# MathThyMod/GP_emu_UQSA

Measured on AMD Instinct MI355X. Metric: log-marginal-likelihood evals/sec at n=16384 d=10 fp64; 1/2/4/8 GPU, higher is better.
Workload: dtype f64

## Files before the change

gp_emu_uqsa_amd/csrc/gpemu.hip:

```cpp
#include <hip/hip_runtime.h>

#include <algorithm>
#include <array>
#include <atomic>
#include <map>
#include <cmath>
#include <cstdio>
#include <cstdlib>
#include <cstring>
#include <limits>
#include <string>
#include <vector>

#include "../../include/gpemu.h"
#include "gpemu_kernels.hpp"
#include "gpemu_gemm_sched.hpp"
#include "gpemu_small.hpp"
#include "gpemu_tiny.hpp"
#include "gpemu_snb.hpp"
#include "gpemu_ozaki.hpp"
#include "gpemu_pivchol.hpp"
#include "gpemu_postgrad.hpp"
#include "gpemu_postmean.hpp"
#include "gpemu_postgroup.hpp"
// ... 11 lines not shown

enum AdhocSlot {
  ADHOC_POST_V = ADHOC_DESC_BASE + 0,
  ADHOC_COV = ADHOC_DESC_BASE + 1,
  ADHOC_NOISE = ADHOC_DESC_BASE + 3,
  ADHOC_PIVCHOL = ADHOC_DESC_BASE + 4,
  ADHOC_POST_U = ADHOC_DESC_BASE + 5,
  ADHOC_TEST = ADHOC_DESC_BASE + 8,
  ADHOC_BENCH = ADHOC_DESC_BASE + 16,
};

struct Plan {
  long long n_pad = 0;
  const double* a_ptr = nullptr;
  const double* b_ptr = nullptr;
  std::vector<int> fused, fused_aug;
  std::vector<int> trtri;
  std::vector<std::vector<std::array<int, 3>>> tri_pairs;
  int lauum = -1;
  bool aug = false;
  std::vector<int> grp, grp_aug;
  int split_h = 0, aug_mid = -1;
  std::vector<int> sfused, sfused_aug, sgrp, sgrp_aug;
  std::vector<GemmLaunch> launches;
  std::vector<GemmProb> probs;
  std::vector<unsigned> tiles;
};

constexpr int FACT_FLAG_INTS = 6;

constexpr int OZ_CHOL_MIN = 8192;


struct Fact {
  long long n_pad = 0;
  int NB = 0;
  double* A = nullptr;
  double* B = nullptr;
  size_t cap = 0;
  double* logdet = nullptr;
  int* flags = nullptr;
  int* tflags = nullptr;
  bool aug = false;
  double* Faug = nullptr;
  double* part = nullptr;
  int* tcnt = nullptr;
  bool xdone = false;
  int desc_base = 0;
  Plan plan;
};

}

struct gpe_ctx {
  int device = 0;
  hipStream_t stream = nullptr;
  std::string err;

  long long n = 0, n_pad = 0;
  int d = 0, q = 0, NB = 0;
  bool has_r = false;

  double* dX = nullptr;
  double* dXw = nullptr;
  double* dF = nullptr;
  double* dr = nullptr;
  Fact tr;
  Fact aux;

  int* dinfo = nullptr;
// ... 26 lines not shown
  double* dtiny = nullptr;
  int tiny_ek = 0, tiny_eg = 0;
  bool tiny_dirty = true;
  double* dsnb = nullptr;
  long long snb_np = 0;
  int snb_hc = 0, snb_mf = 0;
  bool snb_dirty = true;
  double onel_tag = 0.0;
  int oz_on = 1, oz_nmod = OZ_MAXMOD;
  int oz_min_np = 6144;
  int oz_np2 = 0, oz_list_len = 0;
  long long oz_npad = 0;
  OzConst oz_c{};
  int8_t* dozp = nullptr;
  int8_t* dozr = nullptr;
  int* dozx = nullptr;
  unsigned* dozl = nullptr;
  double* dozt = nullptr;
  hipEvent_t ev_oz = nullptr;
  std::vector<OzTriPair> oz_tri;
  int oz_tri_min = 8192;
  double oz_lauum_ops = 0.0;
  int oz_chol = 1, oz_chol_min = OZ_CHOL_MIN;
  OzTriPair oz_chol_q{};
  long long oz_chol_loff = 0;
  int oz_chol_llen = 0;
  double oz_chol_ops = 0.0;
  bool oz_chol_ready = false;
  bool oz_l21_valid = false;
  std::vector<hipEvent_t> oev;
  size_t oev_used = 0;
  double oz_ms = 0.0, oz_launches = 0.0, oz_ops = 0.0, oz_flops64 = 0.0;
  int dbg_skip_wait = -1;
  size_t small_cap = 0;

  double* hpin = nullptr;
  size_t hpin_cap = 0;

  float* dX32 = nullptr;
  size_t x32_cap = 0;
  bool x32_valid = false;
  float* dK32 = nullptr;
  size_t k32_cap = 0;
  hipEvent_t ev_pipe[2] = {nullptr, nullptr};
  int8_t* dpxp = nullptr;
  int* dpxe = nullptr;
// ... 620 lines not shown
        }
        if (i < base.size()) order.push_back(base[i]);
      }
      auto move_to = [&](unsigned code, size_t at) {
        const auto it = std::find(order.begin(), order.end(), code);
        order.erase(it);
        order.insert(order.begin() + std::min(at, order.size()), code);
      };
      if (!rest0.empty() && order.size() > 256 + head) {
        const auto it = std::find(order.begin(), order.end(), rest0.front());
        if ((size_t)(it - order.begin()) > 255 + head) move_to(rest0.front(), 255 + head);
      }
      if (!waits_point_back(fp.data(), order))
        return fail(c, GPE_ERR_HIP, "internal error: group schedule waits on a later tile");
      gidx[o + gb] = (int)pl.launches.size();
      add_launch(pl, GEMM_FUSED, fp, fl, &order);
      pl.launches.back().ticket = flags0 + 3 * NB + gb;
    }
  }
  }
  return GPE_OK;
  };
  CHK(sweep(0, NB, NB, {&pl.fused, &pl.fused_aug, &pl.grp, &pl.grp_aug}));
  for (int s = 2; s / 2 < NB; s *= 2) {
    std::vector<GemmProb> pa, pb;
    const std::vector<std::array<int, 3>> prs = trtri_level_pairs(NB, s);
    double fa = 0.0, fb = 0.0;
    for (const auto& pr : prs) {
      const int t0 = pr[0], h = pr[1], t1 = pr[2];
      const int a = h - t0, b = t1 - h;
      pa.push_back(mkprob(tile(B, t0, t0), ld, tile(A, h, t0), ld, tile(B, t0, h), ld, a, b,
                          a * TILE, G_KBEG_TI, 1.0, 0.0));
      fa += (double)a * T * a * T * b * T;
      pb.push_back(mkprob(tile(B, h, h), ld, tile(B, t0, h), ld, tile(B, h, t0), ld, b, a,
                          b * TILE, G_KEND_TI, -1.0, 0.0));
      fb += (double)b * T * b * T * a * T;
    }
    if (pa.empty()) continue;
    pl.tri_pairs.push_back(prs);
    split_k(pa, F.part, F.tcnt);
    split_k(pb, F.part, F.tcnt);
    pl.trtri.push_back((int)pl.launches.size());
    add_launch(pl, GEMM_AK, pa, fa);
    pl.trtri.push_back((int)pl.launches.size());
    add_launch(pl, GEMM_PLAIN, pb, fb);
  }
  pl.lauum = (int)pl.launches.size();
  {
    const double N = (double)F.n_pad;
    std::vector<GemmProb> lp = {mkprob(B, ld, B, ld, A, ld, NB, NB, (int)F.n_pad, G_CLOWER | G_KBEG_TI, 1.0, 0.0)};
    split_k(lp, F.part, F.tcnt);
    add_launch(pl, GEMM_AK_BK, lp, N * N * N / 3.0);
  }
  const int limit = (F.desc_base == 0) ? AUX_DESC_BASE : ADHOC_DESC_BASE - AUX_DESC_BASE;
  if (const int h = (&F == &c->tr) ? oz_chol_split(c, F) : 0) {
    const size_t nl = pl.launches.size(), np = pl.probs.size(), nt = pl.tiles.size();
    pl.sfused.assign(NB, -1);
    pl.sfused_aug.assign(NB, -1);
    if (c->potrf_group) {
      pl.sgrp.assign(NB, -1);
      if (pl.aug) pl.sgrp_aug.assign(NB, -1);
    }
    const std::array<std::vector<int>*, 4> ix = {&pl.sfused, &pl.sfused_aug, &pl.sgrp, &pl.sgrp_aug};
    CHK(sweep(0, h, NB, ix));
    CHK(sweep(h, NB - h, NB - h, ix));
    if (pl.aug) {
      pl.aug_mid = (int)pl.launches.size();
      add_launch(pl, GEMM_PLAIN, {mkprob(F.Faug, TILE, tile(A, h, 0), ld, F.Faug + (long long)h * TILE * TILE, TILE, 1, NB - h,
                                h * TILE, 0, -1.0, 1.0)}, 0.0);
    }
    pl.split_h = h;
    if ((int)pl.probs.size() > limit) {
      pl.launches.resize(nl);
      pl.probs.resize(np);
      pl.tiles.resize(nt);
      pl.split_h = 0;
      pl.aug_mid = -1;
    }
  }
  if ((int)pl.probs.size() > limit) return fail(c, GPE_ERR_UNSUPPORTED, "GEMM schedule too large");
  for (auto& L : pl.launches) L.first += F.desc_base;
  HIPCHK(c, hipMemcpy(c->dprobs + F.desc_base, pl.probs.data(), pl.probs.size() * sizeof(GemmProb),
                      hipMemcpyHostToDevice));
  const size_t half = pl.tiles.size() + 1;
  const size_t need = 2 * half;
  const bool regrow = need > c->tiles_cap;
  CHK(grow_buf(c, &c->dtiles, &c->tiles_cap, need));
  if (regrow) {
    Fact& other = (&F == &c->tr) ? c->aux : c->tr;
    other.plan = Plan();
  }
  const size_t base = (F.desc_base == 0) ? 0 : c->tiles_cap / 2;
  if (pl.tiles.size() > c->tiles_cap / 2) return fail(c, GPE_ERR_STATE, "tile list overflow");
  for (auto& L : pl.launches)
    if (L.list >= 0) L.list += (long long)base;
  if (!pl.tiles.empty())
    HIPCHK(c, hipMemcpy(c->dtiles + base, pl.tiles.data(), pl.tiles.size() * sizeof(unsigned),
                        hipMemcpyHostToDevice));
  return GPE_OK;
}
// ... 56 lines not shown
    *coff = 1.0;
    *cdiag = predict ? 1.0 + nu * nu : 1.0;
  } else {
    *coff = 1.0 - nu;
    *cdiag = predict ? 1.0 : 1.0 - nu;
  }
}

int kbuild(gpe_ctx* c, int kernel, double nu, double s2, double rscale) {
  PairArgs a;
  a.xr = c->dXw; a.xc = c->dXw; a.out = c->tr.A; a.ld = c->n_pad;
  a.d = c->d; a.nr_valid = (int)c->n; a.nc_valid = (int)c->n;
  a.mt = c->NB; a.nt = c->NB; a.mode = 1 | 2;
  double coff, cdiag;
  kernel_consts(kernel, nu, true, &coff, &cdiag);
  a.s2 = s2; a.coff = coff; a.cdiag = cdiag;
  a.rscale = rscale; a.r = (c->has_r && rscale != 0.0) ? c->dr : nullptr;
  a.fam = kernel_fam(kernel);
  return launch_pairs(c, a, c->NB * (c->NB + 1) / 2);
}

int oz_prepare(gpe_ctx* c, Fact& F);
int chol_schur(gpe_ctx* c, Fact& F, hipStream_t st, bool with_aug);

int potrf(gpe_ctx* c, Fact& F, bool with_aug = false, bool split = false) {
  CHK(build_plan(c, F));
  const int hs = split ? F.plan.split_h : 0;
  if (hs) CHK(oz_prepare(c, F));
  const Plan& pl = F.plan;
  if (hs != (split ? pl.split_h : 0)) return fail(c, GPE_ERR_STATE, "internal error: split plan changed");
  const int NB = F.NB;
  HIPCHK(c, hipMemsetAsync(F.flags, 0, FACT_FLAG_INTS * (size_t)NB * sizeof(int), c->stream));
  F.xdone = false;
  const bool wa = with_aug && pl.aug;
  const bool grp = c->potrf_group &&
                   (c->potrf_mode == 1 || (c->potrf_mode == 0 && g_inflight[c->device & 63].load() <= 1));
  const std::vector<int>& fidx = hs ? (grp ? (wa ? pl.sgrp_aug : pl.sgrp) : (wa ? pl.sfused_aug : pl.sfused))
                                    : (grp ? (wa ? pl.grp_aug : pl.grp) : (wa ? pl.fused_aug : pl.fused));
  if (c->chol_prio) {
    HIPCHK(c, hipEventRecord(c->ev_fork, c->stream));
    HIPCHK(c, hipStreamWaitEvent(c->stream2, c->ev_fork, 0));
    for (int t = 0; t < NB; ++t) {
      if (hs && t == hs) CHK(chol_schur(c, F, c->stream2, wa));
      if (fidx[t] >= 0) CHK(launch_gemm_range(c, pl.launches[fidx[t]], c->stream2));
    }
    HIPCHK(c, hipEventRecord(c->ev_join, c->stream2));
    HIPCHK(c, hipStreamWaitEvent(c->stream, c->ev_join, 0));
    return GPE_OK;
  }
#ifdef GEMM_TTRACE
  if (const char* es = std::getenv("GPEMU_DEBUG_STOP_STEP")) {
    const int stop = std::atoi(es);
    for (int t = 0; t <= stop && t < NB; ++t)
      if (fidx[t] >= 0) CHK(launch_gemm_range(c, pl.launches[fidx[t]]));
    HIPCHK(c, hipStreamSynchronize(c->stream));
    return fail(c, GPE_ERR_STATE, "debug stop after Cholesky launch " + std::to_string(stop));
  }
#endif
  for (int t = 0; t < NB; ++t) {
    if (hs && t == hs) CHK(chol_schur(c, F, c->stream, wa));
    if (fidx[t] >= 0) CHK(launch_gemm_range(c, pl.launches[fidx[t]]));
  }
  return GPE_OK;
}

void ev_rec(gpe_ctx* c, int i);

int lauum(gpe_ctx* c, Fact& F) {
  CHK(build_plan(c, F));
  return launch_gemm_range(c, F.plan.launches[F.plan.lauum]);
}

int ensure_xdiag(gpe_ctx* c, Fact& F) {
  if (F.xdone) return GPE_OK;
  hipLaunchKernelGGL(k_xasm, dim3(F.NB), dim3(256), DB_LDS_DOUBLES * sizeof(double), c->stream, F.A, F.B,
                     (long long)F.n_pad);
  HIPCHK(c, hipGetLastError());
  F.xdone = true;
  return GPE_OK;
}

int trtri_pair_ozaki(gpe_ctx* c, Fact& F, int t0, int h, int t1, int l21);
int oz_l21_ahead(gpe_ctx* c, Fact& F, int t0, int h, int t1);
bool oz_tri_level(const gpe_ctx* c, const std::vector<std::array<int, 3>>& prs);

int trtri(gpe_ctx* c, Fact& F, bool ozaki = false) {
  CHK(build_plan(c, F));
  CHK(ensure_xdiag(c, F));
  const Plan& pl = F.plan;
  int first = -1;
  for (size_t lv = 0; lv < pl.tri_pairs.size() && ozaki && first < 0; ++lv)
    if (oz_tri_level(c, pl.tri_pairs[lv])) first = (int)lv;
  bool have = false;
  if (first >= 0) {
    const auto& pr = pl.tri_pairs[first][0];
    have = c->oz_l21_valid && &F == &c->tr && pl.split_h > 0 && pr[0] == 0 && pr[1] == pl.split_h && pr[2] == F.NB;
    if (!have) CHK(oz_l21_ahead(c, F, pr[0], pr[1], pr[2]));
  }
  for (size_t lv = 0; lv < pl.tri_pairs.size(); ++lv) {
    if (ozaki && oz_tri_level(c, pl.tri_pairs[lv])) {
      for (size_t i = 0; i < pl.tri_pairs[lv].size(); ++i) {
        const auto& pr = pl.tri_pairs[lv][i];
        CHK(trtri_pair_ozaki(c, F, pr[0], pr[1], pr[2], ((int)lv == first && i == 0) ? (have ? 2 : 1) : 0));
      }
      continue;
    }
    CHK(launch_gemm_range(c, pl.launches[pl.trtri[2 * lv]]));
    CHK(launch_gemm_range(c, pl.launches[pl.trtri[2 * lv + 1]]));
  }
  return GPE_OK;
}

int skinny(gpe_ctx* c, bool transposed, const double* M, long long ldm, int ntr, int nit,
           bool lower, const double* R, long long ldr, int P, double* Y, long long ldy) {
  if (P > SK_PMAX) {
    for (int c0 = 0; c0 < P; c0 += SK_PMAX)
      CHK(skinny(c, transposed, M, ldm, ntr, nit, lower, R + (long long)c0 * ldr, ldr, std::min(SK_PMAX, P - c0),
                 Y + (long long)c0 * ldy, ldy));
    return GPE_OK;
  }
  const int kext = lower ? std::max(ntr, nit) : ntr;
  const int want = (256 + nit - 1) / nit;
  const int chk = std::max(1, std::min(SK_CH, (kext + want - 1) / want));
  const int nch = (kext + chk - 1) / chk;
  const long long rows = (long long)nit * TILE;
  CHK(grow_buf(c, &c->dskp, &c->skp_cap, (size_t)nch * rows * P));
  SkinnyArgs a;
  a.M = M; a.ldm = ldm; a.R = R; a.ldr = ldr; a.part = c->dskp; a.ldp = rows;
  a.pstride = rows * P; a.P = P; a.ntr = ntr; a.lower = lower ? 1 : 0; a.nit = nit;
  a.abort_flag = c->dinfo;
  a.chk = chk;
  dim3 grid(nit * nch);
// ... 122 lines not shown
int z_from_factor(gpe_ctx* c);
int trsv_lower(gpe_ctx* c, Fact& F, const double* R, long long ldr, int P, double* Y, long long ldy);

int factor_and_invert(gpe_ctx* c, int kernel, const double* delta, double nu, double s2,
                      double rscale, bool invert = true, bool objective = false) {
  c->linv_valid = false;
  c->oz_l21_valid = false;
  HIPCHK(c, hipStreamSynchronize(c->stream2));
  HIPCHK(c, hipMemsetAsync(c->dinfo, 0, sizeof(int), c->stream));
  CHK(build_plan(c, c->tr));
  ev_rec(c, 0);
  CHK(scale_training(c, delta));
  CHK(kbuild(c, kernel, nu, s2, rscale));
  const int P = c->q + 1;
  c->zaug_valid = !invert && c->tr.plan.aug && P <= TILE;
  if (c->zaug_valid) {
    const long long tot = c->n_pad * TILE;
    hipLaunchKernelGGL(k_aug_init, dim3((unsigned)((tot + 255) / 256)), dim3(256), 0, c->stream, c->dF,
                       c->n_pad, P, c->n_pad, c->tr.Faug);
    HIPCHK(c, hipGetLastError());
  }
  ev_rec(c, 1);
  CHK(build_plan(c, c->tr));
  CHK(potrf(c, c->tr, c->zaug_valid, objective && (invert || c->oz_chol >= 2)));
  if (kernel_fam(kernel) != FAM_GAUSS) {
    double coff, cdiag;
    kernel_consts(kernel, nu, true, &coff, &cdiag);
    const double floor_rel = 4.0 * (double)c->n_pad * std::numeric_limits<double>::epsilon();
    const double* r = (c->has_r && rscale != 0.0) ? c->dr : nullptr;
    hipLaunchKernelGGL(k_pivot_floor, dim3((unsigned)((c->n + 255) / 256)), dim3(256), 0, c->stream, c->tr.A,
                       c->n_pad, (int)c->n, floor_rel, s2 * cdiag, r, rscale, c->dinfo);
    HIPCHK(c, hipGetLastError());
  }
  ev_rec(c, 2);
  if (invert) {
    CHK(trtri(c, c->tr, true));
    c->linv_valid = true;
  }
  CHK(z_from_factor(c));
  ev_rec(c, 3);
  return GPE_OK;
}

int z_from_factor(gpe_ctx* c) {
  const int P = c->q + 1;
  const long long np = c->n_pad;
  if (c->zaug_valid) {
// ... 159 lines not shown
  return nullptr;
}

int oz_l21(gpe_ctx* c, Fact& F, const OzTriPair& q, hipStream_t st) {
  c->oz_l21_valid = false;
  oz_operand(st, c->oz_c, q.l21(F.A + (long long)q.h * TILE + (long long)q.t0 * TILE * F.n_pad, F.n_pad), q.Pb, q.Pa,
             c->dozx, c->dozp);
  HIPCHK(c, hipGetLastError());
  return GPE_OK;
}

int oz_l21_ahead(gpe_ctx* c, Fact& F, int t0, int h, int t1) {
  CHK(oz_prepare(c, F));
  const OzTriPair* q = oz_pair(c, t0, h, t1);
  if (!q) return fail(c, GPE_ERR_STATE, "internal error: TRTRI pair without an int8 plan");
  if (!c->ev_oz) HIPCHK(c, hipEventCreateWithFlags(&c->ev_oz, hipEventDisableTiming));
  HIPCHK(c, hipEventRecord(c->ev_fork, c->stream));
  HIPCHK(c, hipStreamWaitEvent(c->stream2, c->ev_fork, 0));
  CHK(oz_l21(c, F, *q, c->stream2));
  HIPCHK(c, hipEventRecord(c->ev_oz, c->stream2));
  return GPE_OK;
}

int trtri_pair_ozaki(gpe_ctx* c, Fact& F, int t0, int h, int t1, int l21) {
  CHK(oz_prepare(c, F));
  const OzTriPair* qp = oz_pair(c, t0, h, t1);
  if (!qp) return fail(c, GPE_ERR_STATE, "internal error: TRTRI pair without an int8 plan");
  const long long ld = F.n_pad;
  auto tile = [&](double* M, int i, int j) { return M + (long long)i * TILE + (long long)j * TILE * ld; };
  if (l21 == 1) HIPCHK(c, hipStreamWaitEvent(c->stream, c->ev_oz, 0));
  c->oz_l21_valid = false;
  int rc = GPE_OK;
  oz_tri_pair_launches(c->stream, c->oz_c, *qp, c->dozl, tile(F.A, h, t0), tile(F.B, t0, t0), tile(F.B, h, h),
                       tile(F.B, h, t0), ld, c->dozt, c->dozp, c->dozr, c->dozx, l21 != 0,
                       [&](const OzProduct& p, double ops, double fl) {
                         if (rc == GPE_OK) rc = oz_gemm_crt(c, c->oz_c, p, ops, fl);
                       });
  CHK(rc);
  HIPCHK(c, hipGetLastError());
  return GPE_OK;
}

}

bool create_priority_stream(hipStream_t* st) {
  int lo = 0, hi = 0;
  if (hipDeviceGetStreamPriorityRange(&lo, &hi) != hipSuccess) return false;
  return hipStreamCreateWithPriority(st, hipStreamNonBlocking, hi) == hipSuccess;
}

extern "C" {

#ifdef GEMM_TRACE
int gpe_debug_trace(uint64_t* out, int32_t n) {
  if (n > 8 * 4096) n = 8 * 4096;
  return hipMemcpyFromSymbol(out, HIP_SYMBOL(gemm_trace), (size_t)n * 8) == hipSuccess ? 0 : -2;
}
#endif

#ifdef GEMM_TTRACE
// ... 50 lines not shown
  {
    const char* ea = std::getenv("GPEMU_AUG");
    c->tr.aug = !(ea && std::string(ea) == "0");
  }
  {
    const char* e2 = std::getenv("GPEMU_POTRF");
    if (e2) {
      const std::string m(e2);
      c->potrf_group = m == "group" || m == "auto";
      c->potrf_mode = m == "group" ? 1 : (m == "auto" ? 0 : 2);
    }
    if (const char* eg = std::getenv("GPEMU_GROUP_P0")) c->grp_p0 = std::max(1, std::atoi(eg));
    if (const char* eg = std::getenv("GPEMU_GROUP_STRIDE")) c->grp_stride = std::max(0, std::atoi(eg));
    if (const char* ep = std::getenv("GPEMU_CHOL_PRIO")) c->chol_prio = std::atoi(ep) != 0;
    if (const char* et = std::getenv("GPEMU_TINY")) c->tiny = std::atoi(et) != 0;
    if (const char* ed = std::getenv("GPEMU_DEBUG_SKIP_WAIT")) c->dbg_skip_wait = std::atoi(ed);
    if (const char* em = std::getenv("GPEMU_MEAN_CHUNK")) c->mean_chunk = std::max(1, std::atoi(em) / 128) * 128LL;
    if (const char* eo = std::getenv("GPEMU_OZAKI")) c->oz_on = std::atoi(eo) != 0;
    if (const char* en = std::getenv("GPEMU_OZAKI_MIN_NP")) c->oz_min_np = std::max(512, std::atoi(en));
    if (const char* em = std::getenv("GPEMU_OZAKI_MODULI")) c->oz_nmod = std::max(8, std::min(OZ_MAXMOD, std::atoi(em)));
    if (const char* et = std::getenv("GPEMU_OZAKI_TRI_MIN")) c->oz_tri_min = std::max(512, std::atoi(et));
    if (const char* ec = std::getenv("GPEMU_OZAKI_CHOL")) c->oz_chol = std::max(0, std::min(3, std::atoi(ec)));
    if (const char* ec = std::getenv("GPEMU_OZAKI_CHOL_MIN")) c->oz_chol_min = std::max(256, std::atoi(ec));
    if (const char* es = std::getenv("GPEMU_POTRF_SB")) {
      c->potrf_sb = std::max(1, std::min(8, std::atoi(es)));
      if (const char* colon = std::strchr(es, ':')) c->potrf_sb_min = std::max(0, std::atoi(colon + 1));
    }
    if (const char* e3 = std::getenv("GPEMU_POTRF_W")) {
      c->potrf_groups.clear();
      std::string spec(e3);
      size_t pos = 0;
      while (pos < spec.size()) {
        size_t end = spec.find(',', pos);
        if (end == std::string::npos) end = spec.size();
        const std::string item = spec.substr(pos, end - pos);
        const size_t colon = item.find(':');
        const int w = std::atoi(item.substr(0, colon).c_str());
        const int lim = colon == std::string::npos ? 0 : std::atoi(item.substr(colon + 1).c_str());
        if (w >= 1 && w <= 8) c->potrf_groups.push_back({w, lim});
        pos = end + 1;
      }
    }
  }
  if (hipSetDevice(device) != hipSuccess || hipStreamCreateWithFlags(&c->stream, hipStreamNonBlocking) != hipSuccess ||
      !create_priority_stream(&c->stream2) ||
      hipEventCreateWithFlags(&c->ev_fork, hipEventDisableTiming) != hipSuccess ||
      hipEventCreateWithFlags(&c->ev_join, hipEventDisableTiming) != hipSuccess ||
      hipEventCreateWithFlags(&c->ev_host, hipEventDisableTiming) != hipSuccess) {
    g_create_error = "failed to initialise device/stream";
    delete c;
    return nullptr;
  }
  bool ok = dalloc(c, &c->dinfo, 12) == GPE_OK && dalloc(c, &c->dprobs, MAX_PROBS) == GPE_OK &&
            ensure_shape_bufs(c, GPE_MAX_DIMS, GPE_MAX_COLS) == GPE_OK;
  for (int i = 0; i < 16 && ok; ++i) ok = hipEventCreate(&c->ev[i]) == hipSuccess;
  if (ok) {
    const int gl = G_LDS_DOUBLES * (int)sizeof(double);
    ok = hipFuncSetAttribute((const void*)k_gemm<false, false, false, true>, hipFuncAttributeMaxDynamicSharedMemorySize, gl) == hipSuccess &&
         hipFuncSetAttribute((const void*)k_gemm<true, false, false, true>, hipFuncAttributeMaxDynamicSharedMemorySize, gl) == hipSuccess &&
         hipFuncSetAttribute((const void*)k_gemm<true, true, false, true>, hipFuncAttributeMaxDynamicSharedMemorySize, gl) == hipSuccess &&
         hipFuncSetAttribute((const void*)k_gemm<false, true, false, true>, hipFuncAttributeMaxDynamicSharedMemorySize, gl) == hipSuccess &&
         hipFuncSetAttribute((const void*)k_gemm<false, false, true, true>, hipFuncAttributeMaxDynamicSharedMemorySize, gl) == hipSuccess &&
         hipFuncSetAttribute((const void*)k_gemm<false, false>, hipFuncAttributeMaxDynamicSharedMemorySize, gl) == hipSuccess &&
         hipFuncSetAttribute((const void*)k_gemm<true, false>, hipFuncAttributeMaxDynamicSharedMemorySize, gl) == hipSuccess &&
         hipFuncSetAttribute((const void*)k_gemm<true, true>, hipFuncAttributeMaxDynamicSharedMemorySize, gl) == hipSuccess &&
         hipFuncSetAttribute((const void*)k_gemm<false, true>, hipFuncAttributeMaxDynamicSharedMemorySize, gl) == hipSuccess &&
         hipFuncSetAttribute((const void*)k_gemm<false, false, true>, hipFuncAttributeMaxDynamicSharedMemorySize, gl) == hipSuccess &&
         hipFuncSetAttribute((const void*)k_xasm, hipFuncAttributeMaxDynamicSharedMemorySize,
                             (int)(DB_LDS_DOUBLES * sizeof(double))) == hipSuccess;
    const int tl = (G_LDS_LAUNCH_DOUBLES + 2 * TILE * TINY_ZP) * (int)sizeof(double);
// ... 32 lines not shown
    if (F->part) hipFree(F->part);
    if (F->tcnt) hipFree(F->tcnt);
  }
  if (c->tr.tflags) hipFree(c->tr.tflags);
  if (c->dozp) hipFree(c->dozp);
  if (c->dozr) hipFree(c->dozr);
  if (c->dozx) hipFree(c->dozx);
  if (c->dozl) hipFree(c->dozl);
  if (c->dozt) hipFree(c->dozt);
  if (c->ev_oz) hipEventDestroy(c->ev_oz);
  for (hipEvent_t e : c->oev) hipEventDestroy(e);
  if (c->tr.Faug) hipFree(c->tr.Faug);
  if (c->aux.tflags) hipFree(c->aux.tflags);
  if (c->dprobs) hipFree(c->dprobs);
  if (c->dtiles) hipFree(c->dtiles);
  if (c->hpin) hipHostFree(c->hpin);
  for (auto& e : c->ev)
    if (e) hipEventDestroy(e);
  for (auto& e : c->gev) (void)hipEventDestroy(e);
  if (c->ev_fork) (void)hipEventDestroy(c->ev_fork);
  for (hipEvent_t e : c->ev_pipe)
    if (e) (void)hipEventDestroy(e);
  if (c->ev_join) (void)hipEventDestroy(c->ev_join);
  if (c->ev_host) (void)hipEventDestroy(c->ev_host);
  if (c->stream2) {
    (void)hipStreamSynchronize(c->stream2);
    (void)hipStreamDestroy(c->stream2);
  }
  if (c->stream) (void)hipStreamDestroy(c->stream);
  delete c;
}

const char* gpe_last_error(const gpe_ctx* c) {
  if (!c) return g_create_error.c_str();
  return c->err.c_str();
}

int gpe_set_data(gpe_ctx* c, int64_t n, int32_t d, int32_t q, const double* X, const double* f,
                 const double* H, const double* r) {
  if (!c) return GPE_ERR_ARG;
  if (n <= 0 || d <= 0 || q <= 0 || !X || !f || !H) return fail(c, GPE_ERR_ARG, "bad data arguments");
  if (n > (1LL << 20)) return fail(c, GPE_ERR_UNSUPPORTED, "n too large");
  HIPCHK(c, hipSetDevice(c->device));
  HIPCHK(c, hipStreamSynchronize(c->stream));
  CHK(ensure_shape_bufs(c, d, q + 1));
  const long long n_pad = ((n + TILE - 1) / TILE) * TILE;
// ... 59 lines not shown
  return GPE_OK;
}

int gpe_gemm_stats(gpe_ctx* c, double* ms_out, double* launches_out, double* flops_out) {
  if (!c) return GPE_ERR_ARG;
  if (ms_out) *ms_out = c->gemm_ms;
  if (launches_out) *launches_out = c->gemm_launches;
  if (flops_out) *flops_out = c->gemm_flops;
  return GPE_OK;
}

int tiny_objective(gpe_ctx* c, bool gp4ml, int kernel, const double* hp, int n_hp, bool fitnug, double nu,
                   double s2, double rscale, bool want_grad, double* llh_out, double* grad_out, double* sigma2_out) {
  const int d = c->d, q = c->q, P = q + 1;
  TinyArgs a;
  for (int k = 0; k < d; ++k) {
    if (!(hp[k] > 0.0) && !(hp[k] < 0.0))
      return fail(c, GPE_NOT_PD, "length scale delta[" + std::to_string(k) + "] is zero or NaN");
    a.invd[k] = 1.0 / hp[k];
  }
  for (int k = d; k < TINY_DM; ++k) a.invd[k] = 0.0;
  c->linv_valid = false;
  c->zaug_valid = false;
  c->tr.xdone = false;
  HIPCHK(c, hipStreamSynchronize(c->stream2));
  constexpr size_t tiny_doubles = 36 * DB_BS + TILE * 32;
  if (!c->dtiny) CHK(dalloc(c, &c->dtiny, tiny_doubles));
  CHK(ensure_pinned(c, (size_t)P * P + 2 * d + 64 + TINY_NH * 64));
  if (c->tiny_dirty || c->tiny_ek > (1 << 26)) {
    HIPCHK(c, hipMemsetAsync(c->dinfo + 1, 0, (TINY_SYNC_INTS + 1) * sizeof(int), c->stream));
    c->tiny_ek = c->tiny_eg = 0;
    c->tiny_dirty = false;
  }
  ev_rec(c, 0);
  a.X = c->dX; a.F = c->dF;
  a.r = (c->has_r && rscale != 0.0) ? c->dr : nullptr;
  a.rdiag = (gp4ml && !kernel_alt(kernel) && c->has_r) ? c->dr : nullptr;
  a.xw = c->dXw; a.L = c->tr.A; a.Xo = c->tr.B; a.Z = c->dZ; a.small = c->hpin; a.abort_flag = c->dinfo + 1 + TINY_SYNC_INTS;
  a.K = c->tr.A; a.Xp = c->dtiny; a.Wg = c->dtiny + 36 * DB_BS; a.sync = c->dinfo + 1;
  a.n = (int)c->n; a.d = d; a.P = P; a.want_grad = want_grad ? 1 : 0; a.mucm = gp4ml ? 0 : 1;
  a.ek = ++c->tiny_ek;
  a.eg = want_grad ? ++c->tiny_eg : c->tiny_eg;
  a.s2 = s2; a.rscale = rscale;
  a.dbg_skip = c->dbg_skip_wait;
  a.tag = ++c->onel_tag;
  kernel_consts(kernel, nu, true, &a.coff, &a.cdiag);
  a.floor_rel = 4.0 * (double)c->n_pad * std::numeric_limits<double>::epsilon();
// ... 63 lines not shown
    HIPCHK(c, hipStreamSynchronize(c->stream));
    float ms = 0.f;
    (void)hipEventElapsedTime(&ms, c->ev[0], c->ev[7]);
    for (int i = 0; i < 8; ++i) c->phase_ms[i] = 0.0;
    c->phase_ms[6] = ms;
  }
  c->tiny_dirty = false;
  return GPE_OK;
}

int snb_objective(gpe_ctx* c, bool gp4ml, int kernel, const double* hp, int n_hp, bool fitnug, double nu,
                  double s2, double rscale, bool want_grad, double* llh_out, double* grad_out, double* sigma2_out) {
  const int d = c->d, q = c->q, P = q + 1, NB = c->NB;
  const long long np = c->n_pad;
  SnbArgs a;
  for (int k = 0; k < d; ++k) {
    if (!(hp[k] > 0.0) && !(hp[k] < 0.0))
      return fail(c, GPE_NOT_PD, "length scale delta[" + std::to_string(k) + "] is zero or NaN");
    a.invd[k] = 1.0 / hp[k];
  }
  for (int k = d; k < TINY_DM; ++k) a.invd[k] = 0.0;
  c->linv_valid = false;
  c->zaug_valid = false;
  c->tr.xdone = false;
  HIPCHK(c, hipStreamSynchronize(c->stream2));
  if (c->snb_np != np) {
    c->snb_np = 0;
    CHK(dalloc(c, &c->dsnb, (size_t)np * np + 3 * 32 * (size_t)np + TINY_DM * TINY_ZP + TILE * TILE));
    c->snb_np = np;
  }
  CHK(ensure_pinned(c, (size_t)P * P + NB + 2 * d + 64 + SNB_NH * 64));
  if (c->snb_dirty || c->snb_hc > (1 << 24)) {
    HIPCHK(c, hipMemsetAsync(c->dinfo + 8, 0, (SNB_SYNC_INTS + 1) * sizeof(int), c->stream));
    c->snb_hc = c->snb_mf = 0;
    c->snb_dirty = false;
  }
  ev_rec(c, 0);
  a.X = c->dX; a.F = c->dF;
  a.r = (c->has_r && rscale != 0.0) ? c->dr : nullptr;
  a.rdiag = (gp4ml && !kernel_alt(kernel) && c->has_r) ? c->dr : nullptr;
  a.xw = c->dXw; a.A = c->tr.A; a.Lb = c->tr.B; a.Xt = c->dsnb;
  a.Zt = a.Xt + np * np; a.Zo = a.Zt + 32 * np; a.Wg = a.Zo + 32 * np; a.T2g = a.Wg + 32 * np;
  a.Xscr = a.T2g + TINY_DM * TINY_ZP;
  a.small = c->hpin; a.sync = c->dinfo + 8; a.abort_flag = c->dinfo + 8 + SNB_SYNC_INTS;
  a.n = (int)c->n; a.np = (int)np; a.NB = NB; a.d = d; a.P = P; a.want_grad = want_grad ? 1 : 0;
  a.mucm = gp4ml ? 0 : 1;
  a.hcb = c->snb_hc; a.mfb = c->snb_mf;
// ... 1973 lines not shown
```

gp_emu_uqsa_amd/csrc/gpemu_gemm_sched.hpp:

```cpp
#pragma once

#include <algorithm>
#include <cstring>
#include <map>
#include <vector>

#include "gpemu_kernels.hpp"

namespace gpe {

enum GemmKind : int {
  GEMM_PLAIN = 0,
  GEMM_AK = 1,
  GEMM_AK_BK = 2,
  GEMM_BK = 3,
  GEMM_FUSED = 4,
};
struct GemmInstance { bool ak, bk, fused; };
constexpr GemmInstance gemm_instance(GemmKind k) {
  return {k == GEMM_AK || k == GEMM_AK_BK, k == GEMM_BK || k == GEMM_AK_BK, k == GEMM_FUSED};
}
constexpr GemmKind gemm_kind(bool ak, bool bk) { return ak ? (bk ? GEMM_AK_BK : GEMM_AK) : (bk ? GEMM_BK : GEMM_PLAIN); }

struct GemmLaunch {
// ... 29 lines not shown
  GemmLaunch L;
  L.kind = kind;
  L.first = (int)probs.size();
  L.flops = flops;
  return L;
}

inline void push_prob(GemmLaunch& L, std::vector<GemmProb>& probs, GemmProb p, bool cdef_ok) {
  p.tile_begin = L.tiles;
  p.ntiles = prob_tiles(p);
  L.tiles += p.ntiles;
  ++L.count;
  L.cdef = L.cdef || (cdef_ok && gemm_cdef(p));
  probs.push_back(p);
}

inline void set_list(GemmLaunch& L, std::vector<unsigned>& tiles, const std::vector<unsigned>& order) {
  L.list = (long long)tiles.size();
  L.tiles = (int)order.size();
  tiles.insert(tiles.end(), order.begin(), order.end());
}

constexpr int SPLIT_SLOTS = 512;
inline void split_k(std::vector<GemmProb>& probs, double* part, int* tcnt) {
#ifdef GPE_NO_SPLITK
  return;
#endif
  int T = 0, kmax = 0;
  for (const GemmProb& p : probs) {
    if (p.beta != 0.0 || p.ksplit > 1) return;
    T += prob_tiles(p);
    kmax = std::max(kmax, p.K);
  }
  if (T <= 0 || T >= 256) return;
  const int ks = std::min({8, SPLIT_SLOTS / T, kmax / 64});
  if (ks < 2) return;
  int off = 0;
  for (GemmProb& p : probs) {
    const int tl = prob_tiles(p);
    p.ksplit = ks;
    p.part = part + (size_t)off * ks * TILE * TILE;
    p.tcnt = tcnt + off;
    off += tl;
  }
}

inline std::vector<unsigned> xcd_order(const GemmProb* probs, const std::vector<unsigned>& tiles,
                                       const std::vector<unsigned>& placed = {}) {
  struct Row { double tw = 0.0; int at = 0, n = 0; };
  int np = 0;
  for (unsigned code : tiles) np = std::max(np, (int)(code >> 24) + 1);
  std::vector<int> row0(np + 1, 0);
  for (int p = 0; p < np; ++p) row0[p + 1] = row0[p] + std::max(probs[p].mt, 0);
  std::vector<Row> rows(row0[np]);
  const auto row_of = [&](unsigned code) -> Row& { return rows[row0[code >> 24] + ((code >> 12) & 0xfff)]; };
  for (unsigned code : tiles) ++row_of(code).n;
// ... 134 lines not shown
```

gp_emu_uqsa_amd/csrc/gpemu_ozaki.hpp:

```cpp
#pragma once
#include <algorithm>
#include <array>
#include <cmath>
#include <cstdlib>
#include <cstring>
#include <type_traits>
#include <utility>
#include <vector>

namespace gpe {

constexpr int OZ_T = 256;
constexpr int OZ_SK = 64;
constexpr int OZ_NBUF = 4;
constexpr int OZ_OPND = OZ_T * OZ_SK;
constexpr int OZ_LDS = OZ_NBUF * 2 * OZ_OPND;
constexpr int OZ_MAXMOD = 16;
constexpr int OZ_MAX_K = (1 << 17) - 128;

struct OzConst {
  int m[OZ_MAXMOD];
  int c16[OZ_MAXMOD];
  float inv[OZ_MAXMOD];
  double rhi[OZ_MAXMOD];
// ... 640 lines not shown
  const OzShape& s = p.s;
  const int ntj = s.tri ? 0 : s.ntj;
  const OzGemm g{p.a, p.b, p.list, p.list_len, s.K, s.kbeg, s.kend, s.tri, ntj, p.res, p.res_bytes, s.kdiv, s.ti0};
  const OzOut& o = p.out;
  const OzCrt r{p.res, p.res_bytes, s.tri, ntj, o.exr, o.exc, o.C, o.ldc, o.rows, o.cols, o.lower128, o.alpha, s.ti0, o.acc};
  hipError_t e;
  if (e0 && (e = hipEventRecord(e0, st)) != hipSuccess) return e;
  hipLaunchKernelGGL(k_oz_gemm, dim3((unsigned)(k.nmod * g.list_len)), dim3(256), OZ_LDS, st, g, k);
  if (e1 && (e = hipEventRecord(e1, st)) != hipSuccess) return e;
  hipLaunchKernelGGL(k_oz_crt, dim3((unsigned)(s.tiles() * 16)), dim3(256), 0, st, r, k);
  return hipGetLastError();
}

inline std::vector<std::array<int, 3>> trtri_level_pairs(int NB, int s) {
  std::vector<std::array<int, 3>> prs;
  for (int t0 = 0; t0 < NB; t0 += s) {
    const int h = t0 + s / 2;
    if (h >= NB) continue;
    prs.push_back({t0, h, std::min(t0 + s, NB)});
  }
  return prs;
}

struct OzTriPair {
  int t0, h, t1, Ra, Rb, Pa, Pb;
  long long la_off, lb_off;
  int la_len, lb_len;
  double ops_a, ops_b;
  OzShape shape_a() const { return OzShape::rect(Pb / OZ_T, Pa / OZ_T, Pa, 2, 0); }
  OzShape shape_b() const { return OzShape::rect(Pb / OZ_T, Pa / OZ_T, Pb, 0, 1); }
  OzShape shape_schur() const { return OzShape::lower(Pb / OZ_T, 0, Pa, 0); }
  size_t planes_bytes(int N) const { return (size_t)N * Pa * (Pa + Pb); }
  size_t resid_bytes(int N) const { return (size_t)N * shape_a().res_bytes(); }
  OzSrc l21(const double* L21, long long ld) const { return {L21, ld, Rb, Ra, 0, true}; }
};
inline OzTriPair oz_tri_pair_plan(int t0, int h, int t1, int N, std::vector<unsigned>& lists) {
  OzTriPair q;
  q.t0 = t0; q.h = h; q.t1 = t1;
  q.Ra = (h - t0) * TILE;
  q.Rb = (t1 - h) * TILE;
  q.Pa = (q.Ra + OZ_T - 1) / OZ_T * OZ_T;
  q.Pb = (q.Rb + OZ_T - 1) / OZ_T * OZ_T;
  const std::vector<unsigned> la = q.shape_a().list(), lb = q.shape_b().list();
  q.ops_a = q.shape_a().ops(N);
  q.ops_b = q.shape_b().ops(N);
  q.la_off = (long long)lists.size();
  q.la_len = (int)la.size();
  lists.insert(lists.end(), la.begin(), la.end());
  q.lb_off = (long long)lists.size();
  q.lb_len = (int)lb.size();
  lists.insert(lists.end(), lb.begin(), lb.end());
  return q;
}

template <class GC>
void oz_tri_pair_launches(hipStream_t st, const OzConst& k, const OzTriPair& q, const unsigned* lists, const double* L21,
                          const double* X11, const double* X22, double* X21, long long ld, double* T, int8_t* planes,
                          int8_t* res, int* ex, bool l21_done, GC gc) {
  int* exA = ex;
  int* exB = ex + q.Pb;
  int8_t* PA = planes;
  const long long rb = q.shape_a().res_bytes();
  {
    const long long pA = (long long)q.Pb * q.Pa, pB = (long long)q.Pa * q.Pa;
    int8_t* PB = planes + (size_t)k.nmod * pA;
    if (!l21_done) oz_operand(st, k, q.l21(L21, ld), q.Pb, q.Pa, exA, PA);
    oz_operand(st, k, OzSrc{X11, ld, q.Ra, q.Ra, 1, false}, q.Pa, q.Pa, exB, PB);
    gc(OzProduct{q.shape_a(), OzOpnd{PA, pA, q.Pa, 0}, OzOpnd{PB, pB, q.Pa, 0}, lists + q.la_off, q.la_len, res, rb,
                 OzOut{exA, exB, T, (long long)q.Pb, q.Rb, q.Ra, 0, 1.0}},
       q.ops_a, (double)q.Ra * q.Ra * q.Rb);
  }
  {
    const long long pA = (long long)q.Pb * q.Pb, pB = (long long)q.Pa * q.Pb;
    int8_t* PB = planes + (size_t)k.nmod * pA;
    const OzSrc x22{X22, ld, q.Rb, q.Rb, 2, true}, t{T, (long long)q.Pb, q.Ra, q.Rb, 0, false};
    oz_operand_exp(st, k, x22, q.Pb, exA);
    oz_operand_exp(st, k, t, q.Pa, exB);
    oz_operand_split(st, k, x22, q.Pb, q.Pb, exA, PA);
    oz_operand_split(st, k, t, q.Pa, q.Pb, exB, PB);
    gc(OzProduct{q.shape_b(), OzOpnd{PA, pA, q.Pb, 0}, OzOpnd{PB, pB, q.Pb, 0}, lists + q.lb_off, q.lb_len, res, rb,
                 OzOut{exA, exB, X21, ld, q.Rb, q.Ra, 0, -1.0}},
       q.ops_b, (double)q.Rb * q.Rb * q.Ra);
  }
}

}
```

Measured before the change: 18.77.

## Start TRTRI on the factored top-left block while Schur update runs

```diff
diff --git a/gp_emu_uqsa_amd/csrc/gpemu.hip b/gp_emu_uqsa_amd/csrc/gpemu.hip
--- a/gp_emu_uqsa_amd/csrc/gpemu.hip
+++ b/gp_emu_uqsa_amd/csrc/gpemu.hip
@@ -57,6 +57,8 @@
   std::vector<int> grp, grp_aug;
   int split_h = 0, aug_mid = -1;
   std::vector<int> sfused, sfused_aug, sgrp, sgrp_aug;
+  bool sides = false;
+  std::vector<std::array<int, 4>> trtri_side;
   std::vector<GemmLaunch> launches;
   std::vector<GemmProb> probs;
   std::vector<unsigned> tiles;
@@ -80,7 +82,11 @@
   double* Faug = nullptr;
   double* part = nullptr;
   int* tcnt = nullptr;
-  bool xdone = false;
+  bool xdone[2] = {false, false};
+  int xh = 0;
+  int x11 = 0;
+  bool t_ahead = false;
+  void xclear(int h = 0) { xdone[0] = xdone[1] = t_ahead = false; x11 = 0; xh = h; }
   int desc_base = 0;
   Plan plan;
 };
@@ -153,6 +159,8 @@
   int oz_tri_min = 8192;
   double oz_lauum_ops = 0.0;
   int oz_chol = 1, oz_chol_min = OZ_CHOL_MIN;
+  int tri_ahead_on = 1;
+  hipEvent_t ev_l11 = nullptr, ev_schur = nullptr;
   OzTriPair oz_chol_q{};
   long long oz_chol_loff = 0;
   int oz_chol_llen = 0;
@@ -819,20 +827,22 @@
   return GPE_OK;
   };
   CHK(sweep(0, NB, NB, {&pl.fused, &pl.fused_aug, &pl.grp, &pl.grp_aug}));
+  auto tri_pair = [&](const std::array<int, 3>& pr, std::vector<GemmProb>& pa, std::vector<GemmProb>& pb, double& fa,
+                      double& fb) {
+    const int t0 = pr[0], h = pr[1], t1 = pr[2];
+    const int a = h - t0, b = t1 - h;
+    pa.push_back(mkprob(tile(B, t0, t0), ld, tile(A, h, t0), ld, tile(B, t0, h), ld, a, b,
+                        a * TILE, G_KBEG_TI, 1.0, 0.0));
+    fa += (double)a * T * a * T * b * T;
+    pb.push_back(mkprob(tile(B, h, h), ld, tile(B, t0, h), ld, tile(B, h, t0), ld, b, a,
+                        b * TILE, G_KEND_TI, -1.0, 0.0));
+    fb += (double)b * T * b * T * a * T;
+  };
   for (int s = 2; s / 2 < NB; s *= 2) {
     std::vector<GemmProb> pa, pb;
     const std::vector<std::array<int, 3>> prs = trtri_level_pairs(NB, s);
     double fa = 0.0, fb = 0.0;
-    for (const auto& pr : prs) {
-      const int t0 = pr[0], h = pr[1], t1 = pr[2];
-      const int a = h - t0, b = t1 - h;
-      pa.push_back(mkprob(tile(B, t0, t0), ld, tile(A, h, t0), ld, tile(B, t0, h), ld, a, b,
-                          a * TILE, G_KBEG_TI, 1.0, 0.0));
-      fa += (double)a * T * a * T * b * T;
-      pb.push_back(mkprob(tile(B, h, h), ld, tile(B, t0, h), ld, tile(B, h, t0), ld, b, a,
-                          b * TILE, G_KEND_TI, -1.0, 0.0));
-      fb += (double)b * T * b * T * a * T;
-    }
+    for (const auto& pr : prs) tri_pair(pr, pa, pb, fa, fb);
     if (pa.empty()) continue;
     pl.tri_pairs.push_back(prs);
     split_k(pa, F.part, F.tcnt);
@@ -873,6 +883,38 @@
       pl.tiles.resize(nt);
       pl.split_h = 0;
       pl.aug_mid = -1;
+    }
+    if (pl.split_h) {
+      const size_t nl1 = pl.launches.size(), np1 = pl.probs.size(), nt1 = pl.tiles.size();
+      for (size_t lv = 0; lv < pl.tri_pairs.size(); ++lv) {
+        std::array<int, 4> side = {-1, -1, -1, -1};
+        std::vector<GemmProb> wa, wb;
+        double f0 = 0.0, f1 = 0.0;
+        for (const auto& pr : pl.tri_pairs[lv]) tri_pair(pr, wa, wb, f0, f1);
+        int ta = 0, tb = 0, ka = 0, kb = 0;
+        for (const GemmProb& q : wa) { ta += prob_tiles(q); ka = std::max(ka, q.K); }
+        for (const GemmProb& q : wb) { tb += prob_tiles(q); kb = std::max(kb, q.K); }
+        for (int sd = 0; sd < 2; ++sd) {
+          std::vector<GemmProb> pa, pb;
+          double fa = 0.0, fb = 0.0;
+          for (const auto& pr : trtri_side_pairs(pl.tri_pairs[lv], h, sd)) tri_pair(pr, pa, pb, fa, fb);
+          if (pa.empty()) continue;
+          split_k(pa, F.part, F.tcnt, ta, ka);
+          split_k(pb, F.part, F.tcnt, tb, kb);
+          side[2 * sd] = (int)pl.launches.size();
+          add_launch(pl, GEMM_AK, pa, fa);
+          side[2 * sd + 1] = (int)pl.launches.size();
+          add_launch(pl, GEMM_PLAIN, pb, fb);
+        }
+        pl.trtri_side.push_back(side);
+      }
+      pl.sides = true;
+      if ((int)pl.probs.size() > limit) {
+        pl.launches.resize(nl1);
+        pl.probs.resize(np1);
+        pl.tiles.resize(nt1);
+        pl.sides = false;
+      }
     }
   }
   if ((int)pl.probs.size() > limit) return fail(c, GPE_ERR_UNSUPPORTED, "GEMM schedule too large");
@@ -975,8 +1017,9 @@
 
 int oz_prepare(gpe_ctx* c, Fact& F);
 int chol_schur(gpe_ctx* c, Fact& F, hipStream_t st, bool with_aug);
-
-int potrf(gpe_ctx* c, Fact& F, bool with_aug = false, bool split = false) {
+int trtri(gpe_ctx* c, Fact& F, bool ozaki = false, bool ahead = false);
+
+int potrf(gpe_ctx* c, Fact& F, bool with_aug = false, bool split = false, bool ahead = false) {
   CHK(build_plan(c, F));
   const int hs = split ? F.plan.split_h : 0;
   if (hs) CHK(oz_prepare(c, F));
@@ -984,8 +1027,9 @@
   if (hs != (split ? pl.split_h : 0)) return fail(c, GPE_ERR_STATE, "internal error: split plan changed");
   const int NB = F.NB;
   HIPCHK(c, hipMemsetAsync(F.flags, 0, FACT_FLAG_INTS * (size_t)NB * sizeof(int), c->stream));
-  F.xdone = false;
   const bool wa = with_aug && pl.aug;
+  const bool tri_ahead = hs && ahead && pl.sides && c->tri_ahead_on && c->chol_prio;
+  F.xclear(tri_ahead ? hs : 0);
   const bool grp = c->potrf_group &&
                    (c->potrf_mode == 1 || (c->potrf_mode == 0 && g_inflight[c->device & 63].load() <= 1));
   const std::vector<int>& fidx = hs ? (grp ? (wa ? pl.sgrp_aug : pl.sgrp) : (wa ? pl.sfused_aug : pl.sfused))
@@ -994,7 +1038,14 @@
     HIPCHK(c, hipEventRecord(c->ev_fork, c->stream));
     HIPCHK(c, hipStreamWaitEvent(c->stream2, c->ev_fork, 0));
     for (int t = 0; t < NB; ++t) {
-      if (hs && t == hs) CHK(chol_schur(c, F, c->stream2, wa));
+      if (hs && t == hs) {
+        if (tri_ahead) HIPCHK(c, hipEventRecord(c->ev_l11, c->stream2));
+        CHK(chol_schur(c, F, c->stream2, wa));
+        if (tri_ahead) {
+          HIPCHK(c, hipEventRecord(c->ev_schur, c->stream2));
+          CHK(trtri(c, F, true, true));
+        }
+      }
       if (fidx[t] >= 0) CHK(launch_gemm_range(c, pl.launches[fidx[t]], c->stream2));
     }
     HIPCHK(c, hipEventRecord(c->ev_join, c->stream2));
@@ -1024,43 +1075,78 @@
   return launch_gemm_range(c, F.plan.launches[F.plan.lauum]);
 }
 
-int ensure_xdiag(gpe_ctx* c, Fact& F) {
-  if (F.xdone) return GPE_OK;
-  hipLaunchKernelGGL(k_xasm, dim3(F.NB), dim3(256), DB_LDS_DOUBLES * sizeof(double), c->stream, F.A, F.B,
-                     (long long)F.n_pad);
-  HIPCHK(c, hipGetLastError());
-  F.xdone = true;
-  return GPE_OK;
-}
-
-int trtri_pair_ozaki(gpe_ctx* c, Fact& F, int t0, int h, int t1, int l21);
+int ensure_xdiag(gpe_ctx* c, Fact& F, int side = -1) {
+  const bool want0 = side != 1 && !F.xdone[0], want1 = side != 0 && !F.xdone[1];
+  const int a = want0 ? 0 : F.xh, b = want1 ? F.NB : F.xh;
+  if (b > a) {
+    const long long off = (long long)a * TILE * (F.n_pad + 1);
+    hipLaunchKernelGGL(k_xasm, dim3(b - a), dim3(256), DB_LDS_DOUBLES * sizeof(double), c->stream, F.A + off, F.B + off,
+                       (long long)F.n_pad);
+    HIPCHK(c, hipGetLastError());
+  }
+  F.xdone[0] = F.xdone[0] || want0;
+  F.xdone[1] = F.xdone[1] || want1;
+  return GPE_OK;
+}
+
+int trtri_pair_ozaki(gpe_ctx* c, Fact& F, int t0, int h, int t1, int l21, int part = 0);
 int oz_l21_ahead(gpe_ctx* c, Fact& F, int t0, int h, int t1);
 bool oz_tri_level(const gpe_ctx* c, const std::vector<std::array<int, 3>>& prs);
 
-int trtri(gpe_ctx* c, Fact& F, bool ozaki = false) {
+int trtri(gpe_ctx* c, Fact& F, bool ozaki, bool ahead) {
   CHK(build_plan(c, F));
-  CHK(ensure_xdiag(c, F));
   const Plan& pl = F.plan;
+  const int hs = pl.split_h;
+  const bool rest = !ahead && F.x11 > 0 && pl.sides && F.x11 == hs && F.xh == hs;
+  if (ahead && !(pl.sides && F.xh == hs)) return fail(c, GPE_ERR_STATE, "internal error: TRTRI by side without its plan");
+  const int side = ahead ? 0 : (rest ? 1 : -1);
+  const auto is_top = [&](size_t lv) { return side >= 0 && pl.tri_pairs[lv][0][0] < hs && pl.tri_pairs[lv][0][2] > hs; };
+  const auto pairs_of = [&](size_t lv, int sd) {
+    return (sd < 0 || is_top(lv)) ? pl.tri_pairs[lv] : trtri_side_pairs(pl.tri_pairs[lv], hs, sd);
+  };
+  const auto int8_level = [&](size_t lv) { return ozaki && oz_tri_level(c, pl.tri_pairs[lv]); };
+  bool int8_side[2] = {false, false}, int8_top = false;
+  for (size_t lv = 0; lv < pl.tri_pairs.size() && side >= 0; ++lv) {
+    if (!int8_level(lv)) continue;
+    if (is_top(lv)) int8_top = true;
+    else for (int sd = 0; sd < 2; ++sd) int8_side[sd] = int8_side[sd] || !pairs_of(lv, sd).empty();
+  }
+  if (ahead) HIPCHK(c, hipStreamWaitEvent(c->stream, int8_side[0] ? c->ev_schur : c->ev_l11, 0));
+  CHK(ensure_xdiag(c, F, side));
   int first = -1;
-  for (size_t lv = 0; lv < pl.tri_pairs.size() && ozaki && first < 0; ++lv)
-    if (oz_tri_level(c, pl.tri_pairs[lv])) first = (int)lv;
+  for (size_t lv = 0; lv < pl.tri_pairs.size() && !ahead && first < 0; ++lv)
+    if (int8_level(lv) && !pairs_of(lv, side).empty() && !(is_top(lv) && F.t_ahead)) first = (int)lv;
   bool have = false;
   if (first >= 0) {
-    const auto& pr = pl.tri_pairs[first][0];
-    have = c->oz_l21_valid && &F == &c->tr && pl.split_h > 0 && pr[0] == 0 && pr[1] == pl.split_h && pr[2] == F.NB;
+    const auto pr = pairs_of((size_t)first, side)[0];
+    have = c->oz_l21_valid && &F == &c->tr && hs > 0 && pr[0] == 0 && pr[1] == hs && pr[2] == F.NB;
     if (!have) CHK(oz_l21_ahead(c, F, pr[0], pr[1], pr[2]));
   }
   for (size_t lv = 0; lv < pl.tri_pairs.size(); ++lv) {
-    if (ozaki && oz_tri_level(c, pl.tri_pairs[lv])) {
-      for (size_t i = 0; i < pl.tri_pairs[lv].size(); ++i) {
-        const auto& pr = pl.tri_pairs[lv][i];
-        CHK(trtri_pair_ozaki(c, F, pr[0], pr[1], pr[2], ((int)lv == first && i == 0) ? (have ? 2 : 1) : 0));
+    const bool top = is_top(lv);
+    if (top && ahead) {
+      if (!int8_top || int8_side[1]) break;
+      HIPCHK(c, hipStreamWaitEvent(c->stream, c->ev_schur, 0));
+      const auto& pr = pl.tri_pairs[lv][0];
+      CHK(trtri_pair_ozaki(c, F, pr[0], pr[1], pr[2], c->oz_l21_valid ? 2 : 0, 1));
+      F.t_ahead = true;
+      break;
+    }
+    const std::vector<std::array<int, 3>> prs = pairs_of(lv, side);
+    if (prs.empty()) continue;
+    if (int8_level(lv)) {
+      for (size_t i = 0; i < prs.size(); ++i) {
+        const auto& pr = prs[i];
+        const int l21 = ((int)lv == first && i == 0) ? (have ? 2 : 1) : 0;
+        CHK(trtri_pair_ozaki(c, F, pr[0], pr[1], pr[2], l21, (top && F.t_ahead) ? 2 : 0));
       }
       continue;
     }
-    CHK(launch_gemm_range(c, pl.launches[pl.trtri[2 * lv]]));
-    CHK(launch_gemm_range(c, pl.launches[pl.trtri[2 * lv + 1]]));
-  }
+    const bool whole = side < 0 || top;
+    CHK(launch_gemm_range(c, pl.launches[whole ? pl.trtri[2 * lv] : pl.trtri_side[lv][2 * side]]));
+    CHK(launch_gemm_range(c, pl.launches[whole ? pl.trtri[2 * lv + 1] : pl.trtri_side[lv][2 * side + 1]]));
+  }
+  if (ahead) F.x11 = hs;
   return GPE_OK;
 }
 
@@ -1229,7 +1315,7 @@
   }
   ev_rec(c, 1);
   CHK(build_plan(c, c->tr));
-  CHK(potrf(c, c->tr, c->zaug_valid, objective && (invert || c->oz_chol >= 2)));
+  CHK(potrf(c, c->tr, c->zaug_valid, objective && (invert || c->oz_chol >= 2), objective && invert));
   if (kernel_fam(kernel) != FAM_GAUSS) {
     double coff, cdiag;
     kernel_consts(kernel, nu, true, &coff, &cdiag);
@@ -1435,20 +1521,20 @@
   return GPE_OK;
 }
 
-int trtri_pair_ozaki(gpe_ctx* c, Fact& F, int t0, int h, int t1, int l21) {
+int trtri_pair_ozaki(gpe_ctx* c, Fact& F, int t0, int h, int t1, int l21, int part) {
   CHK(oz_prepare(c, F));
   const OzTriPair* qp = oz_pair(c, t0, h, t1);
   if (!qp) return fail(c, GPE_ERR_STATE, "internal error: TRTRI pair without an int8 plan");
   const long long ld = F.n_pad;
   auto tile = [&](double* M, int i, int j) { return M + (long long)i * TILE + (long long)j * TILE * ld; };
   if (l21 == 1) HIPCHK(c, hipStreamWaitEvent(c->stream, c->ev_oz, 0));
-  c->oz_l21_valid = false;
+  if (part != 1) c->oz_l21_valid = false;
   int rc = GPE_OK;
   oz_tri_pair_launches(c->stream, c->oz_c, *qp, c->dozl, tile(F.A, h, t0), tile(F.B, t0, t0), tile(F.B, h, h),
                        tile(F.B, h, t0), ld, c->dozt, c->dozp, c->dozr, c->dozx, l21 != 0,
                        [&](const OzProduct& p, double ops, double fl) {
                          if (rc == GPE_OK) rc = oz_gemm_crt(c, c->oz_c, p, ops, fl);
-                       });
+                       }, part);
   CHK(rc);
   HIPCHK(c, hipGetLastError());
   return GPE_OK;
@@ -1545,6 +1631,7 @@
     if (const char* et = std::getenv("GPEMU_OZAKI_TRI_MIN")) c->oz_tri_min = std::max(512, std::atoi(et));
     if (const char* ec = std::getenv("GPEMU_OZAKI_CHOL")) c->oz_chol = std::max(0, std::min(3, std::atoi(ec)));
     if (const char* ec = std::getenv("GPEMU_OZAKI_CHOL_MIN")) c->oz_chol_min = std::max(256, std::atoi(ec));
+    if (const char* ea = std::getenv("GPEMU_TRTRI_AHEAD")) c->tri_ahead_on = std::atoi(ea) != 0;
     if (const char* es = std::getenv("GPEMU_POTRF_SB")) {
       c->potrf_sb = std::max(1, std::min(8, std::atoi(es)));
       if (const char* colon = std::strchr(es, ':')) c->potrf_sb_min = std::max(0, std::atoi(colon + 1));
@@ -1569,6 +1656,8 @@
       !create_priority_stream(&c->stream2) ||
       hipEventCreateWithFlags(&c->ev_fork, hipEventDisableTiming) != hipSuccess ||
       hipEventCreateWithFlags(&c->ev_join, hipEventDisableTiming) != hipSuccess ||
+      hipEventCreateWithFlags(&c->ev_l11, hipEventDisableTiming) != hipSuccess ||
+      hipEventCreateWithFlags(&c->ev_schur, hipEventDisableTiming) != hipSuccess ||
       hipEventCreateWithFlags(&c->ev_host, hipEventDisableTiming) != hipSuccess) {
     g_create_error = "failed to initialise device/stream";
     delete c;
@@ -1647,6 +1736,8 @@
   for (hipEvent_t e : c->ev_pipe)
     if (e) (void)hipEventDestroy(e);
   if (c->ev_join) (void)hipEventDestroy(c->ev_join);
+  if (c->ev_l11) (void)hipEventDestroy(c->ev_l11);
+  if (c->ev_schur) (void)hipEventDestroy(c->ev_schur);
   if (c->ev_host) (void)hipEventDestroy(c->ev_host);
   if (c->stream2) {
     (void)hipStreamSynchronize(c->stream2);
@@ -1752,7 +1843,7 @@
   for (int k = d; k < TINY_DM; ++k) a.invd[k] = 0.0;
   c->linv_valid = false;
   c->zaug_valid = false;
-  c->tr.xdone = false;
+  c->tr.xclear();
   HIPCHK(c, hipStreamSynchronize(c->stream2));
   constexpr size_t tiny_doubles = 36 * DB_BS + TILE * 32;
   if (!c->dtiny) CHK(dalloc(c, &c->dtiny, tiny_doubles));
@@ -1862,7 +1953,7 @@
   for (int k = d; k < TINY_DM; ++k) a.invd[k] = 0.0;
   c->linv_valid = false;
   c->zaug_valid = false;
-  c->tr.xdone = false;
+  c->tr.xclear();
   HIPCHK(c, hipStreamSynchronize(c->stream2));
   if (c->snb_np != np) {
     c->snb_np = 0;
diff --git a/gp_emu_uqsa_amd/csrc/gpemu_gemm_sched.hpp b/gp_emu_uqsa_amd/csrc/gpemu_gemm_sched.hpp
--- a/gp_emu_uqsa_amd/csrc/gpemu_gemm_sched.hpp
+++ b/gp_emu_uqsa_amd/csrc/gpemu_gemm_sched.hpp
@@ -75,7 +75,7 @@
 }
 
 constexpr int SPLIT_SLOTS = 512;
-inline void split_k(std::vector<GemmProb>& probs, double* part, int* tcnt) {
+inline void split_k(std::vector<GemmProb>& probs, double* part, int* tcnt, int t_all = 0, int k_all = 0) {
 #ifdef GPE_NO_SPLITK
   return;
 #endif
@@ -85,6 +85,7 @@
     T += prob_tiles(p);
     kmax = std::max(kmax, p.K);
   }
+  if (t_all > 0) { T = t_all; kmax = k_all; }
   if (T <= 0 || T >= 256) return;
   const int ks = std::min({8, SPLIT_SLOTS / T, kmax / 64});
   if (ks < 2) return;
diff --git a/gp_emu_uqsa_amd/csrc/gpemu_ozaki.hpp b/gp_emu_uqsa_amd/csrc/gpemu_ozaki.hpp
--- a/gp_emu_uqsa_amd/csrc/gpemu_ozaki.hpp
+++ b/gp_emu_uqsa_amd/csrc/gpemu_ozaki.hpp
@@ -686,6 +686,13 @@
   return prs;
 }
 
+inline std::vector<std::array<int, 3>> trtri_side_pairs(const std::vector<std::array<int, 3>>& prs, int hs, int side) {
+  std::vector<std::array<int, 3>> out;
+  for (const auto& pr : prs)
+    if (!(pr[0] < hs && pr[2] > hs) && (pr[0] >= hs) == (side == 1)) out.push_back(pr);
+  return out;
+}
+
 struct OzTriPair {
   int t0, h, t1, Ra, Rb, Pa, Pb;
   long long la_off, lb_off;
@@ -720,12 +727,12 @@
 template <class GC>
 void oz_tri_pair_launches(hipStream_t st, const OzConst& k, const OzTriPair& q, const unsigned* lists, const double* L21,
                           const double* X11, const double* X22, double* X21, long long ld, double* T, int8_t* planes,
-                          int8_t* res, int* ex, bool l21_done, GC gc) {
+                          int8_t* res, int* ex, bool l21_done, GC gc, int part = 0) {
   int* exA = ex;
   int* exB = ex + q.Pb;
   int8_t* PA = planes;
   const long long rb = q.shape_a().res_bytes();
-  {
+  if (part != 2) {
     const long long pA = (long long)q.Pb * q.Pa, pB = (long long)q.Pa * q.Pa;
     int8_t* PB = planes + (size_t)k.nmod * pA;
     if (!l21_done) oz_operand(st, k, q.l21(L21, ld), q.Pb, q.Pa, exA, PA);
@@ -734,7 +741,7 @@
                  OzOut{exA, exB, T, (long long)q.Pb, q.Rb, q.Ra, 0, 1.0}},
        q.ops_a, (double)q.Ra * q.Ra * q.Rb);
   }
-  {
+  if (part != 1) {
     const long long pA = (long long)q.Pb * q.Pb, pB = (long long)q.Pa * q.Pb;
     int8_t* PB = planes + (size_t)k.nmod * pA;
     const OzSrc x22{X22, ld, q.Rb, q.Rb, 2, true}, t{T, (long long)q.Pb, q.Ra, q.Rb, 0, false};
```

After: 19.15 (median of 6 runs). +2.1%, better.
